# SEEDtk/genome.distance

Hardware: NVIDIA B200
Metric: genome pairs/sec all-vs-all k-mer distance (higher is better)
Workload: dtype u64

## Files before the change

### genome/distance_b200/_lib.py

```python
from __future__ import annotations

import ctypes as C
import os

_HERE = os.path.dirname(os.path.abspath(__file__))
LIB_PATH = os.environ.get("GKD_LIB") or os.path.join(_HERE, "libgkd.so")

GKD_OK, GKD_EINVAL, GKD_EIO, GKD_ENOMEM, GKD_ECUDA, GKD_ESTATE = 0, -1, -2, -3, -4, -5
DNA, PROT, RNA = 0, 1, 2
STRAND_BOTH, STRAND_CANONICAL = 0, 1
AMBIG_SKIP, AMBIG_LITERAL = 0, 1
HASH_JAVA_STRING, HASH_MURMUR3 = 0, 1
ABI_VERSION = 2


class GkdConfig(C.Structure):
    _fields_ = [("device", C.c_int32), ("k", C.c_int32), ("alphabet", C.c_int32), ("strand_mode", C.c_int32),
                ("workspace_bytes", C.c_uint64), ("segment_keys", C.c_uint32), ("ambig_policy", C.c_int32),
                ("reserved", C.c_uint32 * 6)]


class GkdPackedSet(C.Structure):
    _fields_ = [("offs_off", C.c_uint64), ("lows_off", C.c_uint64), ("pal_offs_off", C.c_uint64),
                ("pal_lows_off", C.c_uint64), ("n", C.c_uint32), ("n_pal", C.c_uint32), ("level", C.c_uint32),
# ... 64 lines not shown
    "gkd_query_vs_ref": (_i32, [_vp, _vp, _u32, _vp, _u32, _vp, _vp]),
    "gkd_pairs": (_i32, [_vp, _vp, _vp, _u64, _vp, _vp]),
    "gkd_all_vs_all_range_ex": (_i32, [_vp, _u32, _u64, _u64, C.POINTER(GkdOutputs)]),
    "gkd_query_vs_ref_ex": (_i32, [_vp, _vp, _u32, _vp, _u32, C.POINTER(GkdOutputs)]),
    "gkd_pairs_ex": (_i32, [_vp, _vp, _vp, _u64, C.POINTER(GkdOutputs)]),
    "gkd_greedy_reps": (_i32, [_vp, _vp, _u32, _dbl, _vp]),
    "gkd_pair": (_i32, [_vp, _u32, _u32, _pu64, _pu64, _pdbl]),
    "gkd_all_vs_all_range_within": (_i32, [_vp, _u32, _u64, _u64, _dbl, C.POINTER(GkdHits)]),
    "gkd_query_vs_ref_within": (_i32, [_vp, _vp, _u32, _vp, _u32, _dbl, C.POINTER(GkdHits)]),
    "gkd_query_vs_ref_nearest": (_i32, [_vp, _vp, _u32, _vp, _u32, _u32, _dbl, _i32, _vp, _vp, _vp, _vp]),
    "gkd_hash_set": (_i32, [_vp, _u32, _u32, _i32, _vp, _pu32]),
    "gkd_sketch_distances": (_i32, [_vp, _u32, _i32, _vp, _vp, _u64, _vp]),
    "gkd_format_double": (_i32, [_dbl, C.c_char_p, C.c_size_t]),
    "gkd_get_metrics": (_i32, [_vp, C.POINTER(GkdMetrics)]),
    "gkd_stream": (_vp, [_vp]),
    "gkd_synth_dna": (_i32, [_i32, _vp, _u64, _u64, _u32, _u32, _dbl]),
    "gkd_synth_protein": (_i32, [_i32, _vp, _u64, _u64, _u32, _u32, _dbl]),
}

_lib = None


def load() -> C.CDLL:
    global _lib
    if _lib is not None:
        return _lib
    if not os.path.exists(LIB_PATH):
        raise ImportError(f"{LIB_PATH} is missing: build it with `python -c 'import __graft_entry__ as g; g.build()'` "
                          "(genome.distance_b200 has no CPU fallback)")
    lib = C.CDLL(LIB_PATH)
# ... 7 lines not shown
```

### genome/distance_b200/csrc/gkd_api.cu

```cuda
#include <cuda_runtime.h>
#include <nvtx3/nvToolsExt.h>

#include <algorithm>
#include <cmath>
#include <cstdarg>
#include <cstdio>
#include <cstdlib>
#include <cstring>
#include <new>
#include <string>
#include <unordered_map>
#include <vector>

#include "gkd_internal.cuh"

using namespace gkd;

struct FastaPiece {
    const char *ptr;
    uint64_t len;
};
struct FastaRecord {
    std::string label, comment;
    std::vector<FastaPiece> lines;
// ... 503 lines not shown
    GenomeRec &g = c->genomes[id];
    g.packed = p;
    g.arena = arena_idx;
    set_desc_from_packed(g, base);
    g.built = true;
    c->m.keys_unique += p.n;
}

int build_batch_msd(gkd_ctx *c, const std::vector<BatchGenome> &bg, const std::vector<uint32_t> &ids, uint32_t n_tiles,
                    const uint64_t *keys_in, bool *done) {
    *done = false;
    const uint32_t n = (uint32_t)bg.size();
    std::vector<MsdGenome> msd(n);
    uint32_t n_bins = 0, max_p = 0;
    uint64_t bin_keys = 0;
    bool narrow = true;
    for (uint32_t i = 0; i < n; i++) {
        uint32_t p = level_for(bg[i].n_slots, MSD_BIN_AVG);
        if (bg[i].n_slots >= (1u << 18) && c->key_bits > 32) p = std::max<uint32_t>(p, (uint32_t)c->key_bits - 32);
        p = std::min<uint32_t>(std::min<uint32_t>(p, MSD_MAX_P), (uint32_t)c->key_bits);
        const double mean = (double)bg[i].n_slots / (double)(1u << p);
        uint32_t cap = (uint32_t)(mean + 8.0 * std::sqrt(mean) + 64.0);
        cap = std::min<uint32_t>((cap + 3) & ~3u, MSD_BIN_CAP);
        if (mean > MSD_BIN_AVG) return GKD_OK;
        MsdGenome &M = msd[i];
        M = MsdGenome{};
        M.bin_first = n_bins;
        M.p = p;
        M.s = std::min<uint32_t>(MSD_SORT_BITS, (uint32_t)c->key_bits - p);
        M.cap = cap;
        M.bins_off = bin_keys;
        n_bins += 1u << p;
        bin_keys += (uint64_t)cap << p;
        max_p = std::max(max_p, p);
        narrow = narrow && (c->key_bits - (int)p <= 32);
    }
    int rc;
    if ((rc = ensure(c, c->keys_b, std::max<uint64_t>(bin_keys, 16) * 8))) return rc;
    if ((rc = ensure(c, c->msd_genomes, n * sizeof(MsdGenome)))) return rc;
    if ((rc = ensure(c, c->msd_bins32, (uint64_t)n_bins * 4 + 16))) return rc;
    if ((rc = ensure(c, c->msd_bins64, (uint64_t)n_bins * 8))) return rc;
    if ((rc = ensure(c, c->msd_gstat, (uint64_t)n * 12))) return rc;
    MsdPlan mp{};
    mp.n_bins = n_bins;
    mp.max_p = max_p;
    mp.key_bits = c->key_bits;
    mp.bins = (uint64_t *)c->keys_b.p;
    mp.bin_cursor = (uint32_t *)c->msd_bins32.p;
    mp.overflow = mp.bin_cursor + n_bins;
    mp.status = (unsigned long long *)c->msd_bins64.p;
    mp.genome_valid = (uint32_t *)c->msd_gstat.p;
    mp.genome_maxbin = mp.genome_valid + n;
    mp.genome_unique = mp.genome_maxbin + n;
    CK(cudaMemcpyAsync(c->msd_genomes.p, msd.data(), n * sizeof(MsdGenome), cudaMemcpyHostToDevice, c->stream));
    CK(cudaMemsetAsync(mp.bin_cursor, 0, (size_t)n_bins * 4 + 16, c->stream));
    CK(cudaMemsetAsync(mp.status, 0, (size_t)n_bins * 8, c->stream));
    nvtxRangePushA(keys_in ? "gkd kernel 3: partition into bins" : "gkd kernels 2+3: encode + mix + partition into bins");
    CK(launch_encode_scatter((const BatchGenome *)c->batch_genomes.p, n, n_tiles, (const MsdGenome *)c->msd_genomes.p, max_p,
                             c->cfg.alphabet, c->k, c->mix, keys_in, mp.bins, mp.bin_cursor, mp.overflow, c->stream));
    nvtxRangePop();
    CK(launch_msd_totals((const MsdGenome *)c->msd_genomes.p, n, mp, c->stream));
    c->m.launches += 2;
    std::vector<uint32_t> stat(2 * (size_t)n);
    uint32_t overflow = 0;
    CK(cudaMemcpyAsync(stat.data(), mp.genome_valid, 2 * (size_t)n * 4, cudaMemcpyDeviceToHost, c->stream));
    CK(cudaMemcpyAsync(&overflow, mp.overflow, 4, cudaMemcpyDeviceToHost, c->stream));
    CK(cudaEventRecord(c->ev[1], c->stream));
    CK(cudaEventRecord(c->ev[2], c->stream));
    CK(cudaStreamSynchronize(c->stream));
    if (overflow) return GKD_OK;
    const uint64_t lsz = c->low_bits / 8;
    std::vector<gkd_packed_set> packed(n);
    uint64_t cur = 0;
    for (uint32_t i = 0; i < n; i++) {
// ... 40 lines not shown
int sort_and_finish_lsd(gkd_ctx *c, const std::vector<BatchGenome> &bg, const std::vector<uint32_t> &ids, const SortPlan &plan) {
    uint64_t *sorted = nullptr;
    uint32_t passes = 0;
    nvtxRangePushA("gkd kernel 3: LSD radix sort");
    CK(launch_sort((const BatchGenome *)c->batch_genomes.p, plan, &sorted, &passes, c->stream));
    nvtxRangePop();
    c->m.launches += 3ull * passes;
    c->m.sort_passes = passes;
    CK(cudaEventRecord(c->ev[2], c->stream));
    NvtxRange nvtx("gkd kernel 3: unique + bucket tables");
    return finish_batch(c, bg, ids, plan, sorted);
}

bool msd_applies(const gkd_ctx *c) { return c->use_msd && !has_pal_lists(c); }

int plan_batch(gkd_ctx *c, std::vector<BatchGenome> &bg, SortPlan &plan, uint64_t raw_keys, uint32_t n_tiles) {
    int rc;
    if ((rc = ensure(c, c->keys_a, raw_keys * 8))) return rc;
    if ((rc = ensure(c, c->keys_b, raw_keys * 8))) return rc;
    if ((rc = ensure(c, c->tile_hist, (uint64_t)std::max(n_tiles, 1u) * RADIX_BINS * 4))) return rc;
    if ((rc = ensure(c, c->tile_uniq, (uint64_t)std::max(n_tiles, 1u) * 8))) return rc;
    if ((rc = ensure(c, c->genome_counts, bg.size() * 8))) return rc;
    if ((rc = ensure(c, c->batch_genomes, bg.size() * sizeof(BatchGenome)))) return rc;
    CK(cudaMemcpyAsync(c->batch_genomes.p, bg.data(), bg.size() * sizeof(BatchGenome), cudaMemcpyHostToDevice, c->stream));
    plan.n_genomes = (uint32_t)bg.size();
    plan.n_tiles = n_tiles;
    plan.key_bits = c->key_bits;
    plan.keys_a = (uint64_t *)c->keys_a.p;
    plan.keys_b = (uint64_t *)c->keys_b.p;
    plan.tile_hist = (uint32_t *)c->tile_hist.p;
    plan.tile_uniq = (uint64_t *)c->tile_uniq.p;
    plan.genome_counts = (uint64_t *)c->genome_counts.p;
    return GKD_OK;
}

int build_batch(gkd_ctx *c, uint32_t first, uint32_t last) {
    std::vector<BatchGenome> bg;
    std::vector<uint32_t> ids;
    uint64_t raw = 0;
    uint32_t tiles = 0;
    for (uint32_t id = first; id < last; id++) {
        GenomeRec &g = c->genomes[id];
        BatchGenome b;
        b.codes = (const uint64_t *)g.d_codes;
// ... 3 lines not shown
        b.raw_off = raw;
        b.tile_first = tiles;
        b.n_tiles = (b.n_slots + SORT_TILE - 1) / SORT_TILE;
        raw += ((uint64_t)b.n_slots + 15) & ~15ull;
        tiles += b.n_tiles;
        bg.push_back(b);
        ids.push_back(id);
        c->m.kmer_positions += b.n_slots;
    }
    for (uint32_t id = last; id-- > first;)
        if (c->genomes[id].ready) {
            CK(cudaStreamWaitEvent(c->stream, c->genomes[id].ready, 0));
            break;
        }
    SortPlan plan{};
    int rc = plan_batch(c, bg, plan, std::max<uint64_t>(raw, 16), tiles);
    if (rc) return rc;
    CK(cudaEventRecord(c->ev[0], c->stream));
    c->m.keys_sorted += raw;
    bool done = false;
    if (msd_applies(c)) {
        rc = build_batch_msd(c, bg, ids, tiles, nullptr, &done);
        if (rc) return rc;
        plan.keys_b = (uint64_t *)c->keys_b.p;
    }
    if (!done) {
        nvtxRangePushA("gkd kernel 2: canonical encode + mix");
        CK(launch_encode((const BatchGenome *)c->batch_genomes.p, plan.n_genomes, tiles, c->cfg.alphabet, c->k, c->mix,
                         plan.keys_a, c->stream));
        nvtxRangePop();
        if (tiles) c->m.launches++;
        CK(cudaEventRecord(c->ev[1], c->stream));
        rc = sort_and_finish_lsd(c, bg, ids, plan);
        if (rc) return rc;
    }
    CK(cudaEventRecord(c->ev[3], c->stream));
    CK(cudaStreamSynchronize(c->stream));
    c->m.encode_ms += elapsed(c->ev[0], c->ev[1]);
    c->m.sort_ms += elapsed(c->ev[1], c->ev[2]);
    c->m.unique_ms += elapsed(c->ev[2], c->ev[3]);
    return GKD_OK;
// ... 19 lines not shown
    uint32_t tiles = 0;
    const uint64_t k0 = offsets[i0], total = offsets[i1] - k0;
    for (uint32_t i = i0; i < i1; i++) {
        BatchGenome &b = bg[i - i0];
        b.codes = nullptr;
        b.mask = nullptr;
        b.raw_off = offsets[i] - k0;
        b.n_pos = 0;
        b.n_slots = (uint32_t)(offsets[i + 1] - offsets[i]);
        b.tile_first = tiles;
        b.n_tiles = (b.n_slots + SORT_TILE - 1) / SORT_TILE;
        tiles += b.n_tiles;
        ids[i - i0] = id0 + (i - i0);
    }
    SortPlan plan{};
    int rc = plan_batch(c, bg, plan, std::max<uint64_t>(total, 16), tiles);
    if (rc) return rc;
    if (total) {
        CK(cudaMemcpyAsync(plan.keys_a, keys + k0, total * 8, cudaMemcpyDefault, c->stream));
        if (!on_device) c->m.h2d_bytes += total * 8;
        CK(launch_mix_keys(plan.keys_a, total, c->mix, c->stream));
        c->m.launches++;
    }
    for (uint32_t i = i0; i < i1; i++) c->genomes.push_back(GenomeRec());
    bool done = false;
    rc = GKD_OK;
    if (msd_applies(c)) {
        rc = build_batch_msd(c, bg, ids, tiles, plan.keys_a, &done);
        plan.keys_b = (uint64_t *)c->keys_b.p;
    }
    if (!rc && !done) rc = sort_and_finish_lsd(c, bg, ids, plan);
// ... 805 lines not shown

int gkd_export_set(gkd_ctx *c, uint32_t id, uint64_t *keys, uint64_t cap, uint64_t *n) {
    CHECK_CTX(c);
    int rc = check_built(c, id);
    if (rc) return rc;
    const SetDesc &d = c->genomes[id].desc;
    if (n) *n = d.main.n;
    if (!keys) return GKD_OK;
    if (cap < d.main.n) return fail(c, GKD_EINVAL, "export buffer holds %llu keys, set has %u", (unsigned long long)cap, d.main.n);
    if (d.main.n == 0) return GKD_OK;
    CK(cudaSetDevice(c->cfg.device));
    ABI_GUARD_BEGIN
    std::vector<BatchGenome> bg(1);
    bg[0] = BatchGenome{nullptr, nullptr, 0, 0, d.main.n, 0, (d.main.n + SORT_TILE - 1) / SORT_TILE};
    SortPlan plan{};
    if ((rc = plan_batch(c, bg, plan, d.main.n, bg[0].n_tiles))) return rc;
    CK(launch_unmix_set(d.main, c->mix, c->low_bits, plan.keys_a, c->stream));
    uint64_t *sorted = nullptr;
    uint32_t passes = 0;
    CK(launch_sort((const BatchGenome *)c->batch_genomes.p, plan, &sorted, &passes, c->stream));
    c->m.launches += 1 + 3ull * passes;
    CK(cudaMemcpyAsync(keys, sorted, (uint64_t)d.main.n * 8, cudaMemcpyDefault, c->stream));
    CK(cudaStreamSynchronize(c->stream));
    c->m.d2h_bytes += (uint64_t)d.main.n * 8;
    return GKD_OK;
    ABI_GUARD_END(c)
}

int gkd_import_sets(gkd_ctx *c, const uint64_t *keys, const uint64_t *offsets, uint32_t n_sets, uint32_t *first_id) {
    CHECK_CTX(c);
    if (first_id) *first_id = (uint32_t)c->genomes.size();
// ... 613 lines not shown
    CK(cudaMemcpyAsync(dist, c->d_dist.p, n_pairs * 8, cudaMemcpyDefault, c->stream));
    CK(cudaStreamSynchronize(c->stream));
    c->m.d2h_bytes += n_pairs * 8;
    return GKD_OK;
    ABI_GUARD_END(c)
}

int gkd_get_metrics(const gkd_ctx *c, gkd_metrics *out) {
    if (!c || !out) return GKD_EINVAL;
    *out = c->m;
    return GKD_OK;
}

void *gkd_stream(const gkd_ctx *c) { return c ? (void *)c->stream : nullptr; }

int gkd_format_double(double v, char *buf, size_t cap) {
    if (std::isnan(v)) return snprintf(buf, cap, "NaN");
    if (std::isinf(v)) return snprintf(buf, cap, v > 0 ? "Infinity" : "-Infinity");
    if (v == 0.0) return snprintf(buf, cap, std::signbit(v) ? "-0.0" : "0.0");
    char tmp[48];
    int prec = 17;
    for (int p = 1; p <= 17; p++) {
        snprintf(tmp, sizeof(tmp), "%.*e", p - 1, v);
        if (strtod(tmp, nullptr) == v) {
            prec = p;
            break;
        }
    }
    snprintf(tmp, sizeof(tmp), "%.*e", prec - 1, v);
    std::string mant;
// ... 45 lines not shown
```

### genome/distance_b200/csrc/gkd_internal.cuh

```cuda
#pragma once

#include <cuda_runtime.h>
#include <stdint.h>

#include "gkd.h"

namespace gkd {

constexpr uint64_t KEY_SENTINEL = 0xFFFFFFFFFFFFFFFFull;

struct MixParams {
    uint64_t mask;
    uint64_t fix;
    int bits;
    int shift;
};

constexpr uint64_t MIX_C1 = 0xff51afd7ed558ccdull, MIX_C2 = 0xc4ceb9fe1a85ec53ull;
constexpr uint64_t MIX_I1 = 0x4f74430c22a54005ull, MIX_I2 = 0x9cb4b2f8129337dbull;

__host__ __device__ inline uint64_t mix_rounds(uint64_t x, uint64_t mask, int s) {
    x ^= x >> s;
    x = (x * MIX_C1) & mask;
    x ^= x >> s;
// ... 130 lines not shown
constexpr uint32_t MSD_MAX_P = 12, MSD_SORT_BITS = 12;
struct MsdGenome {
    uint32_t bin_first;
    uint32_t p;
    uint32_t s;
    uint32_t level;
    uint32_t cap;
    uint32_t pad_;
    uint64_t bins_off;
    void *lows;
    uint32_t *offs;
};
struct MsdPlan {
    uint32_t n_bins, max_p;
    int key_bits;
    uint64_t *bins;
    uint32_t *bin_cursor;
    unsigned long long *status;
    uint32_t *genome_valid, *genome_maxbin, *genome_unique, *overflow;
};
cudaError_t msd_configure();
cudaError_t launch_encode_scatter(const BatchGenome *genomes, uint32_t n_genomes, uint32_t n_tiles, const MsdGenome *msd,
                                  uint32_t max_p, int alphabet, int k, MixParams mix, const uint64_t *keys_in, uint64_t *bins_out,
                                  uint32_t *bin_cursor, uint32_t *overflow, cudaStream_t s);
cudaError_t launch_msd_totals(const MsdGenome *msd, uint32_t n_genomes, const MsdPlan &plan, cudaStream_t s);
cudaError_t launch_msd_binsort(const MsdGenome *msd, uint32_t n_genomes, const MsdPlan &plan, int low_bits, bool narrow,
                               cudaStream_t s);
cudaError_t launch_mix_keys(uint64_t *keys, uint64_t n, MixParams mix, cudaStream_t s);
cudaError_t launch_unmix_set(SubSet set, MixParams mix, int low_bits, uint64_t *keys_out, cudaStream_t s);
cudaError_t launch_fill_u64(uint64_t *dst, uint64_t n, uint64_t value, cudaStream_t s);
struct IsectPlan {
    int low_bits;
    uint32_t tmax;
    uint32_t level_min;
    uint32_t groups_per_item;
    uint32_t items_per_pair;
};
cudaError_t intersect_configure();
uint32_t intersect_default_tmax(int low_bits);
// ... 107 lines not shown
```

### genome/distance_b200/csrc/pack_encode.cu

```cuda
#include "gkd_internal.cuh"

namespace gkd {

__device__ __forceinline__ uint32_t nonzero_bytes(uint32_t v) {
    return (((v & 0x7F7F7F7Fu) + 0x7F7F7F7Fu) | v) & 0x80808080u;
}

__global__ void __launch_bounds__(256) k_pack_dna(const char *__restrict__ text, uint64_t n_pos, uint64_t n_words,
                                                   uint64_t *__restrict__ codes, uint32_t *__restrict__ mask, int rna) {
    uint64_t w = (uint64_t)blockIdx.x * blockDim.x + threadIdx.x;
    if (w >= n_words) return;
    uint64_t p0 = w * PACK_POS_PER_WORD;
    uint32_t x[8];
    const char *src = text + p0;
    if (p0 + 32 <= n_pos && ((reinterpret_cast<uintptr_t>(src) & 15) == 0)) {
        uint4 a = __ldg(reinterpret_cast<const uint4 *>(src));
        uint4 b = __ldg(reinterpret_cast<const uint4 *>(src) + 1);
        x[0] = a.x; x[1] = a.y; x[2] = a.z; x[3] = a.w;
        x[4] = b.x; x[5] = b.y; x[6] = b.z; x[7] = b.w;
    } else {
#pragma unroll
        for (int q = 0; q < 8; q++) {
            uint32_t v = 0;
#pragma unroll
// ... 153 lines not shown
        }
#pragma unroll
        for (int u = 0; u < 4; u++) base[u] = v[u] ? atomicAdd(&cursor[b0 + u * ENC_THREADS], v[u]) : 0u;
#pragma unroll
        for (int u = 0; u < 4; u++)
            if (v[u]) {
                if (base[u] + v[u] > cap) {
                    atomicExch(overflow, 1u);
                    base[u] = 0xFFFFFFFFu;
                }
                s_bin[b0 + u * ENC_THREADS] = base[u];
            }
    }
}

template <int ALPHA>
__global__ void __launch_bounds__(ENC_THREADS, 4)
    k_encode_scatter(const BatchGenome *__restrict__ genomes, uint32_t n_genomes, const MsdGenome *__restrict__ msd, int k,
                     MixParams mix, uint64_t *__restrict__ bins_out, uint32_t *__restrict__ bin_cursor,
                     uint32_t *__restrict__ overflow) {
    extern __shared__ uint32_t s_bin[];
    __shared__ uint32_t s_g;
    if (threadIdx.x == 0) s_g = find_genome(genomes, n_genomes, blockIdx.x);
    __syncthreads();
    const BatchGenome G = genomes[s_g];
    const MsdGenome M = msd[s_g];
    const uint32_t n_bins = 1u << M.p;
    for (uint32_t i = threadIdx.x; i < n_bins; i += ENC_THREADS) s_bin[i] = 0;
    __syncthreads();
    const int shift = mix.bits - (int)M.p;
    const uint32_t my0 = (blockIdx.x - G.tile_first) * ENC_TILE + threadIdx.x * ENC_PER_THREAD;
    uint64_t key[ENC_PER_THREAD];
    uint32_t rank[ENC_PER_THREAD];
#pragma unroll
    for (int j = 0; j < ENC_PER_THREAD; j++) key[j] = KEY_SENTINEL, rank[j] = 0;
    if (my0 < G.n_slots)
        encode_thread<ALPHA>(G, k, mix, my0, [&](int j, uint64_t h) {
            key[j] = h;
            if (h != KEY_SENTINEL) rank[j] = atomicAdd(&s_bin[M.p ? (uint32_t)(h >> shift) : 0u], 1u);
        });
    __syncthreads();
    reserve_bins(s_bin, n_bins, bin_cursor + M.bin_first, M.cap, overflow);
    __syncthreads();
    uint64_t *out = bins_out + M.bins_off;
#pragma unroll
    for (int j = 0; j < ENC_PER_THREAD; j++)
        if (key[j] != KEY_SENTINEL) {
            const uint32_t b = M.p ? (uint32_t)(key[j] >> shift) : 0u;
            const uint32_t base = s_bin[b];
            if (base != 0xFFFFFFFFu) out[(uint64_t)b * M.cap + base + rank[j]] = key[j];
        }
}

__global__ void __launch_bounds__(ENC_THREADS)
    k_keys_scatter(const BatchGenome *__restrict__ genomes, uint32_t n_genomes, const MsdGenome *__restrict__ msd, int key_bits,
                   const uint64_t *__restrict__ in, uint64_t *__restrict__ bins_out, uint32_t *__restrict__ bin_cursor,
                   uint32_t *__restrict__ overflow) {
    extern __shared__ uint32_t s_bin[];
    __shared__ uint32_t s_g;
    if (threadIdx.x == 0) s_g = find_genome(genomes, n_genomes, blockIdx.x);
    __syncthreads();
    const BatchGenome G = genomes[s_g];
    const MsdGenome M = msd[s_g];
    const uint32_t n_bins = 1u << M.p;
    for (uint32_t i = threadIdx.x; i < n_bins; i += ENC_THREADS) s_bin[i] = 0;
    __syncthreads();
    const int shift = key_bits - (int)M.p;
    const uint32_t slot0 = (blockIdx.x - G.tile_first) * ENC_TILE;
    const uint32_t count = min((uint32_t)ENC_TILE, G.n_slots - slot0);
    const uint64_t *src = in + G.raw_off + slot0;
    uint64_t key[ENC_PER_THREAD];
    uint32_t rank[ENC_PER_THREAD];
#pragma unroll
    for (int j = 0; j < ENC_PER_THREAD; j++) {
        const uint32_t idx = j * ENC_THREADS + threadIdx.x;
        key[j] = idx < count ? src[idx] : KEY_SENTINEL;
        rank[j] = 0;
        if (key[j] != KEY_SENTINEL) rank[j] = atomicAdd(&s_bin[M.p ? (uint32_t)(key[j] >> shift) : 0u], 1u);
    }
    __syncthreads();
    reserve_bins(s_bin, n_bins, bin_cursor + M.bin_first, M.cap, overflow);
    __syncthreads();
    uint64_t *out = bins_out + M.bins_off;
#pragma unroll
    for (int j = 0; j < ENC_PER_THREAD; j++)
        if (key[j] != KEY_SENTINEL) {
            const uint32_t b = M.p ? (uint32_t)(key[j] >> shift) : 0u;
            const uint32_t base = s_bin[b];
            if (base != 0xFFFFFFFFu) out[(uint64_t)b * M.cap + base + rank[j]] = key[j];
        }
}

cudaError_t launch_encode(const BatchGenome *genomes, uint32_t n_genomes, uint32_t n_tiles, int alphabet, int k,
                          MixParams mix, uint64_t *keys_out, cudaStream_t s) {
    if (n_tiles == 0) return cudaSuccess;
    if (alphabet == GKD_PROT) k_encode<GKD_PROT><<<n_tiles, ENC_THREADS, 0, s>>>(genomes, n_genomes, k, mix, keys_out);
    else k_encode<GKD_DNA><<<n_tiles, ENC_THREADS, 0, s>>>(genomes, n_genomes, k, mix, keys_out);
    return cudaGetLastError();
}

}

namespace gkd {

cudaError_t launch_encode_scatter(const BatchGenome *genomes, uint32_t n_genomes, uint32_t n_tiles, const MsdGenome *msd,
                                  uint32_t max_p, int alphabet, int k, MixParams mix, const uint64_t *keys_in, uint64_t *bins_out,
                                  uint32_t *bin_cursor, uint32_t *overflow, cudaStream_t s) {
    if (n_tiles == 0) return cudaSuccess;
    const uint32_t smem = (1u << max_p) * 4;
    if (keys_in)
        k_keys_scatter<<<n_tiles, ENC_THREADS, smem, s>>>(genomes, n_genomes, msd, mix.bits, keys_in, bins_out, bin_cursor, overflow);
    else if (alphabet == GKD_PROT)
        k_encode_scatter<GKD_PROT><<<n_tiles, ENC_THREADS, smem, s>>>(genomes, n_genomes, msd, k, mix, bins_out, bin_cursor, overflow);
    else
        k_encode_scatter<GKD_DNA><<<n_tiles, ENC_THREADS, smem, s>>>(genomes, n_genomes, msd, k, mix, bins_out, bin_cursor, overflow);
    return cudaGetLastError();
}

}
```

### genome/distance_b200/csrc/sort_msd.cu

```cuda
#include "gkd_internal.cuh"

namespace gkd {

constexpr int MSD_THREADS = 512;
constexpr int MSD_KPT = (MSD_BIN_CAP + MSD_THREADS - 1) / MSD_THREADS;

__global__ void __launch_bounds__(256)
    k_msd_totals(const MsdGenome *__restrict__ msd, const uint32_t *__restrict__ bin_cursor,
                 uint32_t *__restrict__ genome_valid, uint32_t *__restrict__ genome_maxbin) {
    __shared__ uint32_t s_sum, s_max;
    const MsdGenome M = msd[blockIdx.x];
    if (threadIdx.x == 0) s_sum = 0, s_max = 0;
    __syncthreads();
    uint32_t sum = 0, mx = 0;
    for (uint32_t b = threadIdx.x; b < (1u << M.p); b += 256) {
        const uint32_t v = bin_cursor[M.bin_first + b];
        sum += v;
        mx = v > mx ? v : mx;
    }
    sum = __reduce_add_sync(0xffffffffu, sum);
    mx = __reduce_max_sync(0xffffffffu, mx);
    if ((threadIdx.x & 31) == 0) {
        atomicAdd(&s_sum, sum);
        atomicMax(&s_max, mx);
// ... 20 lines not shown
    for (int w = 0; w < MSD_THREADS / 32; w++) {
        const uint32_t c = s_warp[w];
        if (w < warp) base += c;
        tot += c;
    }
    *total = tot;
    __syncthreads();
    return base + incl - v;
}

constexpr unsigned long long LB_AGG = 1ull << 62, LB_PREFIX = 2ull << 62, LB_MASK = (1ull << 62) - 1;

template <typename KT, typename LowT>
__global__ void __launch_bounds__(MSD_THREADS, 2)
    k_msd_binsort(const MsdGenome *__restrict__ msd, uint32_t n_genomes, int key_bits, const uint32_t *__restrict__ bin_cursor,
                  const uint64_t *__restrict__ bins, unsigned long long *__restrict__ status,
                  uint32_t *__restrict__ genome_unique) {
    extern __shared__ __align__(16) unsigned char s_raw[];
    KT *s_k = reinterpret_cast<KT *>(s_raw);
    KT *s_o = s_k + MSD_BIN_CAP;
    uint32_t *s_cnt = reinterpret_cast<uint32_t *>(s_o + MSD_BIN_CAP);
    uint32_t *s_start = s_cnt + (1u << MSD_SORT_BITS);
    __shared__ uint32_t s_warp[MSD_THREADS / 32];
    __shared__ unsigned long long s_prefix;
    uint32_t lo = 0, hi = n_genomes;
    while (hi - lo > 1) {
        const uint32_t mid = (lo + hi) >> 1;
        if (msd[mid].bin_first <= blockIdx.x) lo = mid;
        else hi = mid;
    }
    const MsdGenome M = msd[lo];
    const uint32_t bin = blockIdx.x - M.bin_first, n_bins = 1u << M.p;
    uint32_t c = bin_cursor[blockIdx.x];
    if (c > M.cap || c > MSD_BIN_CAP) c = 0;
    const uint64_t *src = bins + M.bins_off + (uint64_t)bin * M.cap;
    const int rest = key_bits - (int)M.p;
    const uint64_t rest_mask = rest >= 64 ? ~0ull : ((1ull << rest) - 1ull);
    const uint32_t s = M.s, n_sb = 1u << s;
    const int sb_shift = rest - (int)s;

    for (uint32_t i = threadIdx.x; i < n_sb; i += MSD_THREADS) s_cnt[i] = 0;
    __syncthreads();
    KT kv[MSD_KPT];
    uint32_t meta[MSD_KPT];
    const int rounds = (int)((c + MSD_THREADS - 1) / MSD_THREADS);
    uint64_t raw[MSD_KPT];
#pragma unroll
    for (int j = 0; j < MSD_KPT; j++) {
        if (j >= rounds) break;
        const uint32_t i = j * MSD_THREADS + threadIdx.x;
        raw[j] = i < c ? src[i] : 0ull;
    }
#pragma unroll
    for (int j = 0; j < MSD_KPT; j++) {
        if (j >= rounds) break;
        const uint32_t i = j * MSD_THREADS + threadIdx.x;
        kv[j] = 0;
        meta[j] = 0;
        if (i < c) {
            const uint64_t h = raw[j] & rest_mask;
            const uint32_t sb = s ? (uint32_t)(h >> sb_shift) : 0u;
            kv[j] = (KT)h;
            meta[j] = sb | (atomicAdd(&s_cnt[sb], 1u) << 16);
        }
    }
    __syncthreads();
    {
        constexpr uint32_t SB_PT = (1u << MSD_SORT_BITS) / MSD_THREADS;
        static_assert(SB_PT * MSD_THREADS == (1u << MSD_SORT_BITS) && SB_PT >= 1, "whole sort-buckets per thread");
        const uint32_t a = SB_PT * threadIdx.x;
        uint32_t v[SB_PT], sum = 0, total;
#pragma unroll
        for (uint32_t q = 0; q < SB_PT; q++) {
            v[q] = a + q < n_sb ? s_cnt[a + q] : 0u;
            sum += v[q];
// ... 84 lines not shown
    }
    if (bin == n_bins - 1 && threadIdx.x == 0) {
        M.offs[(size_t)1 << M.level] = prefix + u;
        genome_unique[lo] = prefix + u;
    }
}

template <typename KT>
static constexpr uint32_t binsort_smem() { return 2 * MSD_BIN_CAP * (uint32_t)sizeof(KT) + (2 * (1u << MSD_SORT_BITS) + 8) * 4; }

cudaError_t msd_configure() {
    cudaError_t e;
#define X(KT, LT)                                                                                                  \
    if ((e = cudaFuncSetAttribute(k_msd_binsort<KT, LT>, cudaFuncAttributeMaxDynamicSharedMemorySize, (int)binsort_smem<KT>()))) \
        return e;
    X(uint32_t, uint32_t) X(uint64_t, uint32_t) X(uint64_t, uint64_t)
#undef X
    return cudaSuccess;
}

cudaError_t launch_msd_totals(const MsdGenome *msd, uint32_t n_genomes, const MsdPlan &plan, cudaStream_t s) {
    if (n_genomes == 0) return cudaSuccess;
    k_msd_totals<<<n_genomes, 256, 0, s>>>(msd, plan.bin_cursor, plan.genome_valid, plan.genome_maxbin);
    return cudaGetLastError();
}

cudaError_t launch_msd_binsort(const MsdGenome *msd, uint32_t n_genomes, const MsdPlan &plan, int low_bits, bool narrow,
                               cudaStream_t s) {
    if (plan.n_bins == 0) return cudaSuccess;
    if (low_bits == 32 && narrow)
        k_msd_binsort<uint32_t, uint32_t><<<plan.n_bins, MSD_THREADS, binsort_smem<uint32_t>(), s>>>(
            msd, n_genomes, plan.key_bits, plan.bin_cursor, plan.bins, plan.status, plan.genome_unique);
    else if (low_bits == 32)
        k_msd_binsort<uint64_t, uint32_t><<<plan.n_bins, MSD_THREADS, binsort_smem<uint64_t>(), s>>>(
            msd, n_genomes, plan.key_bits, plan.bin_cursor, plan.bins, plan.status, plan.genome_unique);
    else
        k_msd_binsort<uint64_t, uint64_t><<<plan.n_bins, MSD_THREADS, binsort_smem<uint64_t>(), s>>>(
            msd, n_genomes, plan.key_bits, plan.bin_cursor, plan.bins, plan.status, plan.genome_unique);
    return cudaGetLastError();
}

}
```

### genome/distance_b200/engine.py

```python
from __future__ import annotations

import ctypes as C
from typing import List, Sequence, Tuple

import numpy as np

from . import _lib
from ._lib import (AMBIG_LITERAL, AMBIG_SKIP, DNA, PROT, RNA, STRAND_BOTH, STRAND_CANONICAL, GkdConfig, GkdHits,
                   GkdMetrics, GkdOutputs, GkdPackedSet)

PACKED_DTYPE = np.dtype([("offs_off", "<u8"), ("lows_off", "<u8"), ("pal_offs_off", "<u8"), ("pal_lows_off", "<u8"),
                         ("n", "<u4"), ("n_pal", "<u4"), ("level", "<u4"), ("pal_level", "<u4")])
assert PACKED_DTYPE.itemsize == C.sizeof(GkdPackedSet)


FIRST_HITS_CAP = 1 << 20


def _select(call, pairs: int):
    cap = min(pairs, FIRST_HITS_CAP)
    while True:
        a, b = np.empty(cap, dtype=np.uint32), np.empty(cap, dtype=np.uint32)
        inter, dist = np.empty(cap, dtype=np.uint64), np.empty(cap, dtype=np.float64)
        h = GkdHits(a.ctypes.data, b.ctypes.data, inter.ctypes.data, dist.ctypes.data, cap, 0)
# ... 18 lines not shown
class Engine:

    def __init__(self, k: int = 0, alphabet: int = DNA, strand_mode: int = STRAND_BOTH, device: int = 0,
                 workspace_bytes: int = 0, segment_keys: int = 0, ambig_policy: int = AMBIG_SKIP):
        self._L = _lib.load()
        cfg = GkdConfig(device=device, k=k, alphabet=alphabet, strand_mode=strand_mode,
                        workspace_bytes=workspace_bytes, segment_keys=segment_keys, ambig_policy=ambig_policy)
        h = C.c_void_p()
        rc = self._L.gkd_create(C.byref(h), C.byref(cfg))
        if rc:
            raise GkdError(rc, (self._L.gkd_last_error(None) or b"").decode())
        self._h = h
        self.device = device
        self.alphabet = alphabet
        self._keep: List[object] = []
        self._adopted: List[Tuple[int, object]] = []

    def _ck(self, rc: int):
        if rc:
            raise GkdError(rc, (self._L.gkd_last_error(self._h) or b"").decode())

    def close(self):
        if getattr(self, "_h", None):
            self._L.gkd_destroy(self._h)
            self._h = None

    def __del__(self):
        try:
            self.close()
        except Exception:
# ... 19 lines not shown
            t = x.contiguous()
            return t.data_ptr(), t.numel() * t.element_size(), t
        raise TypeError(f"unsupported sequence type {type(x)}")

    def add(self, contigs) -> int:
        if isinstance(contigs, (str, bytes, bytearray, np.ndarray)) or _is_torch(contigs):
            contigs = [contigs]
        triples = [self._ptr_len(c) for c in contigs]
        n = len(triples)
        ptrs = (C.c_void_p * max(n, 1))(*[t[0] for t in triples])
        lens = (C.c_uint64 * max(n, 1))(*[t[1] for t in triples])
        out = C.c_uint32()
        if any(_is_torch(c) and c.is_cuda for c in contigs):
            import torch

            torch.cuda.synchronize(self.device)
        self._ck(self._L.gkd_add_sequences(self._h, ptrs, lens, n, C.byref(out)))
        self._keep.extend(t[2] for t in triples if _is_torch(t[2]))
        return out.value

    def add_fasta(self, path: str, per_record: bool = True) -> Tuple[int, int]:
        first, n = C.c_uint32(), C.c_uint32()
        self._ck(self._L.gkd_add_fasta_file(self._h, path.encode(), 1 if per_record else 0, C.byref(first), C.byref(n)))
        return first.value, n.value

    def label(self, i: int) -> str:
        return self._L.gkd_label(self._h, i).decode("latin-1")

    def comment(self, i: int) -> str:
        return self._L.gkd_comment(self._h, i).decode("latin-1")

# ... 299 lines not shown
```

### include/gkd.h

```cpp
#ifndef GKD_H
#define GKD_H

#include <stddef.h>
#include <stdint.h>

#ifdef __cplusplus
extern "C" {
#endif

#define GKD_ABI_VERSION 2

typedef enum gkd_status {
    GKD_OK = 0,
    GKD_EINVAL = -1,
    GKD_EIO = -2,
    GKD_ENOMEM = -3,
    GKD_ECUDA = -4,
    GKD_ESTATE = -5
} gkd_status;

typedef enum gkd_alphabet { GKD_DNA = 0, GKD_PROT = 1, GKD_RNA = 2 } gkd_alphabet;

typedef enum gkd_strand_mode { GKD_STRAND_BOTH = 0, GKD_STRAND_CANONICAL = 1 } gkd_strand_mode;

// ... 117 lines not shown
int gkd_group_add_fasta_file(gkd_group *g, const char *path, uint32_t *n_added);
const char *gkd_group_label(const gkd_group *g, uint32_t global_id);
const char *gkd_group_comment(const gkd_group *g, uint32_t global_id);
int gkd_group_build(gkd_group *g);
int gkd_group_all_vs_all(gkd_group *g, uint64_t *inter, double *dist);
int gkd_group_all_vs_all_within(gkd_group *g, double max_dist, gkd_hits *out);

typedef enum gkd_sketch_hash { GKD_HASH_JAVA_STRING = 0, GKD_HASH_MURMUR3 = 1 } gkd_sketch_hash;
int gkd_hash_set(gkd_ctx *ctx, uint32_t id, uint32_t width, int hash, int32_t *out, uint32_t *n_out);
int gkd_sketch_distances(gkd_ctx *ctx, uint32_t width, int hash, const uint32_t *a, const uint32_t *b, uint64_t n_pairs,
                         double *dist);

int gkd_format_double(double v, char *buf, size_t cap);
int gkd_get_metrics(const gkd_ctx *ctx, gkd_metrics *out);
void *gkd_stream(const gkd_ctx *ctx);

int gkd_synth_dna(int device, char *dst, uint64_t len, uint64_t seed, uint32_t family, uint32_t member,
                  double sub_rate);
int gkd_synth_protein(int device, char *dst, uint64_t len, uint64_t seed, uint32_t family, uint32_t member,
                      double sub_rate);

#ifdef __cplusplus
}
#endif
#endif
```

Before: 1.394 million.

## Store narrow MSD bin keys as 32-bit and replace host sync with event wait

When every genome's post-bin remainder fits in 32 bits, the encode/scatter kernels now write only the masked low bits into 32-bit bin buffers, and the binsort kernel reads them as uint32 (a new uint32/uint64 instantiation is added). This halves scatter and binsort global memory traffic and the size of the keys_b allocation, and LSD key buffers are now allocated only when the MSD path does not finish the batch. Separately, adding CUDA-tensor contigs no longer calls a full device synchronize; it records a torch event and makes the library streams wait on it. The risks are correctness in the masking and narrow logic, plus ordering subtleties from the asynchronous handoff.

```diff
diff --git a/genome/distance_b200/_lib.py b/genome/distance_b200/_lib.py
--- a/genome/distance_b200/_lib.py
+++ b/genome/distance_b200/_lib.py
@@ -102,6 +102,7 @@
     "gkd_format_double": (_i32, [_dbl, C.c_char_p, C.c_size_t]),
     "gkd_get_metrics": (_i32, [_vp, C.POINTER(GkdMetrics)]),
     "gkd_stream": (_vp, [_vp]),
+    "gkd_wait_event": (_i32, [_vp, _vp]),
     "gkd_synth_dna": (_i32, [_i32, _vp, _u64, _u64, _u32, _u32, _dbl]),
     "gkd_synth_protein": (_i32, [_i32, _vp, _u64, _u64, _u32, _u32, _dbl]),
 }
diff --git a/genome/distance_b200/csrc/gkd_api.cu b/genome/distance_b200/csrc/gkd_api.cu
--- a/genome/distance_b200/csrc/gkd_api.cu
+++ b/genome/distance_b200/csrc/gkd_api.cu
@@ -541,11 +541,15 @@
     std::vector<MsdGenome> msd(n);
     uint32_t n_bins = 0, max_p = 0;
     uint64_t bin_keys = 0;
-    bool narrow = true;
-    for (uint32_t i = 0; i < n; i++) {
+    auto bin_bits = [&](uint32_t i) {
         uint32_t p = level_for(bg[i].n_slots, MSD_BIN_AVG);
         if (bg[i].n_slots >= (1u << 18) && c->key_bits > 32) p = std::max<uint32_t>(p, (uint32_t)c->key_bits - 32);
-        p = std::min<uint32_t>(std::min<uint32_t>(p, MSD_MAX_P), (uint32_t)c->key_bits);
+        return std::min<uint32_t>(std::min<uint32_t>(p, MSD_MAX_P), (uint32_t)c->key_bits);
+    };
+    bool narrow = true;
+    for (uint32_t i = 0; i < n; i++) narrow = narrow && (c->key_bits - (int)bin_bits(i) <= 32);
+    for (uint32_t i = 0; i < n; i++) {
+        const uint32_t p = bin_bits(i);
         const double mean = (double)bg[i].n_slots / (double)(1u << p);
         uint32_t cap = (uint32_t)(mean + 8.0 * std::sqrt(mean) + 64.0);
         cap = std::min<uint32_t>((cap + 3) & ~3u, MSD_BIN_CAP);
@@ -560,10 +564,9 @@
         n_bins += 1u << p;
         bin_keys += (uint64_t)cap << p;
         max_p = std::max(max_p, p);
-        narrow = narrow && (c->key_bits - (int)p <= 32);
     }
     int rc;
-    if ((rc = ensure(c, c->keys_b, std::max<uint64_t>(bin_keys, 16) * 8))) return rc;
+    if ((rc = ensure(c, c->keys_b, std::max<uint64_t>(bin_keys, 16) * (narrow ? 4 : 8)))) return rc;
     if ((rc = ensure(c, c->msd_genomes, n * sizeof(MsdGenome)))) return rc;
     if ((rc = ensure(c, c->msd_bins32, (uint64_t)n_bins * 4 + 16))) return rc;
     if ((rc = ensure(c, c->msd_bins64, (uint64_t)n_bins * 8))) return rc;
@@ -572,7 +575,7 @@
     mp.n_bins = n_bins;
     mp.max_p = max_p;
     mp.key_bits = c->key_bits;
-    mp.bins = (uint64_t *)c->keys_b.p;
+    mp.bins = c->keys_b.p;
     mp.bin_cursor = (uint32_t *)c->msd_bins32.p;
     mp.overflow = mp.bin_cursor + n_bins;
     mp.status = (unsigned long long *)c->msd_bins64.p;
@@ -584,7 +587,8 @@
     CK(cudaMemsetAsync(mp.status, 0, (size_t)n_bins * 8, c->stream));
     nvtxRangePushA(keys_in ? "gkd kernel 3: partition into bins" : "gkd kernels 2+3: encode + mix + partition into bins");
     CK(launch_encode_scatter((const BatchGenome *)c->batch_genomes.p, n, n_tiles, (const MsdGenome *)c->msd_genomes.p, max_p,
-                             c->cfg.alphabet, c->k, c->mix, keys_in, mp.bins, mp.bin_cursor, mp.overflow, c->stream));
+                             narrow, c->cfg.alphabet, c->k, c->mix, keys_in, c->keys_b.p, mp.bin_cursor, mp.overflow,
+                             c->stream));
     nvtxRangePop();
     CK(launch_msd_totals((const MsdGenome *)c->msd_genomes.p, n, mp, c->stream));
     c->m.launches += 2;
@@ -655,10 +659,17 @@
 
 bool msd_applies(const gkd_ctx *c) { return c->use_msd && !has_pal_lists(c); }
 
-int plan_batch(gkd_ctx *c, std::vector<BatchGenome> &bg, SortPlan &plan, uint64_t raw_keys, uint32_t n_tiles) {
+int plan_lsd_keys(gkd_ctx *c, SortPlan &plan, uint64_t raw_keys) {
     int rc;
     if ((rc = ensure(c, c->keys_a, raw_keys * 8))) return rc;
     if ((rc = ensure(c, c->keys_b, raw_keys * 8))) return rc;
+    plan.keys_a = (uint64_t *)c->keys_a.p;
+    plan.keys_b = (uint64_t *)c->keys_b.p;
+    return GKD_OK;
+}
+
+int plan_batch(gkd_ctx *c, std::vector<BatchGenome> &bg, SortPlan &plan, uint32_t n_tiles) {
+    int rc;
     if ((rc = ensure(c, c->tile_hist, (uint64_t)std::max(n_tiles, 1u) * RADIX_BINS * 4))) return rc;
     if ((rc = ensure(c, c->tile_uniq, (uint64_t)std::max(n_tiles, 1u) * 8))) return rc;
     if ((rc = ensure(c, c->genome_counts, bg.size() * 8))) return rc;
@@ -667,8 +678,6 @@
     plan.n_genomes = (uint32_t)bg.size();
     plan.n_tiles = n_tiles;
     plan.key_bits = c->key_bits;
-    plan.keys_a = (uint64_t *)c->keys_a.p;
-    plan.keys_b = (uint64_t *)c->keys_b.p;
     plan.tile_hist = (uint32_t *)c->tile_hist.p;
     plan.tile_uniq = (uint64_t *)c->tile_uniq.p;
     plan.genome_counts = (uint64_t *)c->genome_counts.p;
@@ -702,7 +711,7 @@
             break;
         }
     SortPlan plan{};
-    int rc = plan_batch(c, bg, plan, std::max<uint64_t>(raw, 16), tiles);
+    int rc = plan_batch(c, bg, plan, tiles);
     if (rc) return rc;
     CK(cudaEventRecord(c->ev[0], c->stream));
     c->m.keys_sorted += raw;
@@ -710,9 +719,9 @@
     if (msd_applies(c)) {
         rc = build_batch_msd(c, bg, ids, tiles, nullptr, &done);
         if (rc) return rc;
-        plan.keys_b = (uint64_t *)c->keys_b.p;
     }
     if (!done) {
+        if ((rc = plan_lsd_keys(c, plan, std::max<uint64_t>(raw, 16)))) return rc;
         nvtxRangePushA("gkd kernel 2: canonical encode + mix");
         CK(launch_encode((const BatchGenome *)c->batch_genomes.p, plan.n_genomes, tiles, c->cfg.alphabet, c->k, c->mix,
                          plan.keys_a, c->stream));
@@ -762,7 +771,8 @@
         ids[i - i0] = id0 + (i - i0);
     }
     SortPlan plan{};
-    int rc = plan_batch(c, bg, plan, std::max<uint64_t>(total, 16), tiles);
+    int rc = plan_batch(c, bg, plan, tiles);
+    if (!rc) rc = plan_lsd_keys(c, plan, std::max<uint64_t>(total, 16));
     if (rc) return rc;
     if (total) {
         CK(cudaMemcpyAsync(plan.keys_a, keys + k0, total * 8, cudaMemcpyDefault, c->stream));
@@ -1598,7 +1608,7 @@
     std::vector<BatchGenome> bg(1);
     bg[0] = BatchGenome{nullptr, nullptr, 0, 0, d.main.n, 0, (d.main.n + SORT_TILE - 1) / SORT_TILE};
     SortPlan plan{};
-    if ((rc = plan_batch(c, bg, plan, d.main.n, bg[0].n_tiles))) return rc;
+    if ((rc = plan_batch(c, bg, plan, bg[0].n_tiles)) || (rc = plan_lsd_keys(c, plan, d.main.n))) return rc;
     CK(launch_unmix_set(d.main, c->mix, c->low_bits, plan.keys_a, c->stream));
     uint64_t *sorted = nullptr;
     uint32_t passes = 0;
@@ -2242,6 +2252,14 @@
 
 void *gkd_stream(const gkd_ctx *c) { return c ? (void *)c->stream : nullptr; }
 
+int gkd_wait_event(gkd_ctx *c, void *event) {
+    if (!c || !event) return GKD_EINVAL;
+    CK(cudaSetDevice(c->cfg.device));
+    CK(cudaStreamWaitEvent(c->copy_stream, (cudaEvent_t)event, 0));
+    CK(cudaStreamWaitEvent(c->stream, (cudaEvent_t)event, 0));
+    return GKD_OK;
+}
+
 int gkd_format_double(double v, char *buf, size_t cap) {
     if (std::isnan(v)) return snprintf(buf, cap, "NaN");
     if (std::isinf(v)) return snprintf(buf, cap, v > 0 ? "Infinity" : "-Infinity");
diff --git a/genome/distance_b200/csrc/gkd_internal.cuh b/genome/distance_b200/csrc/gkd_internal.cuh
--- a/genome/distance_b200/csrc/gkd_internal.cuh
+++ b/genome/distance_b200/csrc/gkd_internal.cuh
@@ -168,15 +168,15 @@
 struct MsdPlan {
     uint32_t n_bins, max_p;
     int key_bits;
-    uint64_t *bins;
+    const void *bins;
     uint32_t *bin_cursor;
     unsigned long long *status;
     uint32_t *genome_valid, *genome_maxbin, *genome_unique, *overflow;
 };
 cudaError_t msd_configure();
 cudaError_t launch_encode_scatter(const BatchGenome *genomes, uint32_t n_genomes, uint32_t n_tiles, const MsdGenome *msd,
-                                  uint32_t max_p, int alphabet, int k, MixParams mix, const uint64_t *keys_in, uint64_t *bins_out,
-                                  uint32_t *bin_cursor, uint32_t *overflow, cudaStream_t s);
+                                  uint32_t max_p, bool narrow, int alphabet, int k, MixParams mix, const uint64_t *keys_in,
+                                  void *bins_out, uint32_t *bin_cursor, uint32_t *overflow, cudaStream_t s);
 cudaError_t launch_msd_totals(const MsdGenome *msd, uint32_t n_genomes, const MsdPlan &plan, cudaStream_t s);
 cudaError_t launch_msd_binsort(const MsdGenome *msd, uint32_t n_genomes, const MsdPlan &plan, int low_bits, bool narrow,
                                cudaStream_t s);
diff --git a/genome/distance_b200/csrc/pack_encode.cu b/genome/distance_b200/csrc/pack_encode.cu
--- a/genome/distance_b200/csrc/pack_encode.cu
+++ b/genome/distance_b200/csrc/pack_encode.cu
@@ -191,10 +191,10 @@
     }
 }
 
-template <int ALPHA>
+template <int ALPHA, typename KT>
 __global__ void __launch_bounds__(ENC_THREADS, 4)
     k_encode_scatter(const BatchGenome *__restrict__ genomes, uint32_t n_genomes, const MsdGenome *__restrict__ msd, int k,
-                     MixParams mix, uint64_t *__restrict__ bins_out, uint32_t *__restrict__ bin_cursor,
+                     MixParams mix, KT *__restrict__ bins_out, uint32_t *__restrict__ bin_cursor,
                      uint32_t *__restrict__ overflow) {
     extern __shared__ uint32_t s_bin[];
     __shared__ uint32_t s_g;
@@ -219,19 +219,21 @@
     __syncthreads();
     reserve_bins(s_bin, n_bins, bin_cursor + M.bin_first, M.cap, overflow);
     __syncthreads();
-    uint64_t *out = bins_out + M.bins_off;
+    const uint64_t rest_mask = shift >= 64 ? ~0ull : ((1ull << shift) - 1ull);
+    KT *out = bins_out + M.bins_off;
 #pragma unroll
     for (int j = 0; j < ENC_PER_THREAD; j++)
         if (key[j] != KEY_SENTINEL) {
             const uint32_t b = M.p ? (uint32_t)(key[j] >> shift) : 0u;
             const uint32_t base = s_bin[b];
-            if (base != 0xFFFFFFFFu) out[(uint64_t)b * M.cap + base + rank[j]] = key[j];
-        }
-}
-
+            if (base != 0xFFFFFFFFu) out[(uint64_t)b * M.cap + base + rank[j]] = (KT)(key[j] & rest_mask);
+        }
+}
+
+template <typename KT>
 __global__ void __launch_bounds__(ENC_THREADS)
     k_keys_scatter(const BatchGenome *__restrict__ genomes, uint32_t n_genomes, const MsdGenome *__restrict__ msd, int key_bits,
-                   const uint64_t *__restrict__ in, uint64_t *__restrict__ bins_out, uint32_t *__restrict__ bin_cursor,
+                   const uint64_t *__restrict__ in, KT *__restrict__ bins_out, uint32_t *__restrict__ bin_cursor,
                    uint32_t *__restrict__ overflow) {
     extern __shared__ uint32_t s_bin[];
     __shared__ uint32_t s_g;
@@ -258,13 +260,14 @@
     __syncthreads();
     reserve_bins(s_bin, n_bins, bin_cursor + M.bin_first, M.cap, overflow);
     __syncthreads();
-    uint64_t *out = bins_out + M.bins_off;
+    const uint64_t rest_mask = shift >= 64 ? ~0ull : ((1ull << shift) - 1ull);
+    KT *out = bins_out + M.bins_off;
 #pragma unroll
     for (int j = 0; j < ENC_PER_THREAD; j++)
         if (key[j] != KEY_SENTINEL) {
             const uint32_t b = M.p ? (uint32_t)(key[j] >> shift) : 0u;
             const uint32_t base = s_bin[b];
-            if (base != 0xFFFFFFFFu) out[(uint64_t)b * M.cap + base + rank[j]] = key[j];
+            if (base != 0xFFFFFFFFu) out[(uint64_t)b * M.cap + base + rank[j]] = (KT)(key[j] & rest_mask);
         }
 }
 
@@ -280,18 +283,29 @@
 
 namespace gkd {
 
-cudaError_t launch_encode_scatter(const BatchGenome *genomes, uint32_t n_genomes, uint32_t n_tiles, const MsdGenome *msd,
-                                  uint32_t max_p, int alphabet, int k, MixParams mix, const uint64_t *keys_in, uint64_t *bins_out,
-                                  uint32_t *bin_cursor, uint32_t *overflow, cudaStream_t s) {
-    if (n_tiles == 0) return cudaSuccess;
+template <typename KT>
+static cudaError_t encode_scatter_t(const BatchGenome *genomes, uint32_t n_genomes, uint32_t n_tiles, const MsdGenome *msd,
+                                    uint32_t max_p, int alphabet, int k, MixParams mix, const uint64_t *keys_in, KT *bins_out,
+                                    uint32_t *bin_cursor, uint32_t *overflow, cudaStream_t s) {
     const uint32_t smem = (1u << max_p) * 4;
     if (keys_in)
-        k_keys_scatter<<<n_tiles, ENC_THREADS, smem, s>>>(genomes, n_genomes, msd, mix.bits, keys_in, bins_out, bin_cursor, overflow);
+        k_keys_scatter<KT><<<n_tiles, ENC_THREADS, smem, s>>>(genomes, n_genomes, msd, mix.bits, keys_in, bins_out, bin_cursor, overflow);
     else if (alphabet == GKD_PROT)
-        k_encode_scatter<GKD_PROT><<<n_tiles, ENC_THREADS, smem, s>>>(genomes, n_genomes, msd, k, mix, bins_out, bin_cursor, overflow);
+        k_encode_scatter<GKD_PROT, KT><<<n_tiles, ENC_THREADS, smem, s>>>(genomes, n_genomes, msd, k, mix, bins_out, bin_cursor, overflow);
     else
-        k_encode_scatter<GKD_DNA><<<n_tiles, ENC_THREADS, smem, s>>>(genomes, n_genomes, msd, k, mix, bins_out, bin_cursor, overflow);
+        k_encode_scatter<GKD_DNA, KT><<<n_tiles, ENC_THREADS, smem, s>>>(genomes, n_genomes, msd, k, mix, bins_out, bin_cursor, overflow);
     return cudaGetLastError();
 }
 
-}
+cudaError_t launch_encode_scatter(const BatchGenome *genomes, uint32_t n_genomes, uint32_t n_tiles, const MsdGenome *msd,
+                                  uint32_t max_p, bool narrow, int alphabet, int k, MixParams mix, const uint64_t *keys_in,
+                                  void *bins_out, uint32_t *bin_cursor, uint32_t *overflow, cudaStream_t s) {
+    if (n_tiles == 0) return cudaSuccess;
+    if (narrow)
+        return encode_scatter_t<uint32_t>(genomes, n_genomes, n_tiles, msd, max_p, alphabet, k, mix, keys_in,
+                                          (uint32_t *)bins_out, bin_cursor, overflow, s);
+    return encode_scatter_t<uint64_t>(genomes, n_genomes, n_tiles, msd, max_p, alphabet, k, mix, keys_in,
+                                      (uint64_t *)bins_out, bin_cursor, overflow, s);
+}
+
+}
diff --git a/genome/distance_b200/csrc/sort_msd.cu b/genome/distance_b200/csrc/sort_msd.cu
--- a/genome/distance_b200/csrc/sort_msd.cu
+++ b/genome/distance_b200/csrc/sort_msd.cu
@@ -58,7 +58,7 @@
 template <typename KT, typename LowT>
 __global__ void __launch_bounds__(MSD_THREADS, 2)
     k_msd_binsort(const MsdGenome *__restrict__ msd, uint32_t n_genomes, int key_bits, const uint32_t *__restrict__ bin_cursor,
-                  const uint64_t *__restrict__ bins, unsigned long long *__restrict__ status,
+                  const KT *__restrict__ bins, unsigned long long *__restrict__ status,
                   uint32_t *__restrict__ genome_unique) {
     extern __shared__ __align__(16) unsigned char s_raw[];
     KT *s_k = reinterpret_cast<KT *>(s_raw);
@@ -77,7 +77,7 @@
     const uint32_t bin = blockIdx.x - M.bin_first, n_bins = 1u << M.p;
     uint32_t c = bin_cursor[blockIdx.x];
     if (c > M.cap || c > MSD_BIN_CAP) c = 0;
-    const uint64_t *src = bins + M.bins_off + (uint64_t)bin * M.cap;
+    const KT *src = bins + M.bins_off + (uint64_t)bin * M.cap;
     const int rest = key_bits - (int)M.p;
     const uint64_t rest_mask = rest >= 64 ? ~0ull : ((1ull << rest) - 1ull);
     const uint32_t s = M.s, n_sb = 1u << s;
@@ -88,12 +88,12 @@
     KT kv[MSD_KPT];
     uint32_t meta[MSD_KPT];
     const int rounds = (int)((c + MSD_THREADS - 1) / MSD_THREADS);
-    uint64_t raw[MSD_KPT];
+    KT raw[MSD_KPT];
 #pragma unroll
     for (int j = 0; j < MSD_KPT; j++) {
         if (j >= rounds) break;
         const uint32_t i = j * MSD_THREADS + threadIdx.x;
-        raw[j] = i < c ? src[i] : 0ull;
+        raw[j] = i < c ? src[i] : (KT)0;
     }
 #pragma unroll
     for (int j = 0; j < MSD_KPT; j++) {
@@ -102,7 +102,7 @@
         kv[j] = 0;
         meta[j] = 0;
         if (i < c) {
-            const uint64_t h = raw[j] & rest_mask;
+            const uint64_t h = (uint64_t)raw[j] & rest_mask;
             const uint32_t sb = s ? (uint32_t)(h >> sb_shift) : 0u;
             kv[j] = (KT)h;
             meta[j] = sb | (atomicAdd(&s_cnt[sb], 1u) << 16);
@@ -217,7 +217,7 @@
 #define X(KT, LT)                                                                                                  \
     if ((e = cudaFuncSetAttribute(k_msd_binsort<KT, LT>, cudaFuncAttributeMaxDynamicSharedMemorySize, (int)binsort_smem<KT>()))) \
         return e;
-    X(uint32_t, uint32_t) X(uint64_t, uint32_t) X(uint64_t, uint64_t)
+    X(uint32_t, uint32_t) X(uint32_t, uint64_t) X(uint64_t, uint32_t) X(uint64_t, uint64_t)
 #undef X
     return cudaSuccess;
 }
@@ -233,13 +233,16 @@
     if (plan.n_bins == 0) return cudaSuccess;
     if (low_bits == 32 && narrow)
         k_msd_binsort<uint32_t, uint32_t><<<plan.n_bins, MSD_THREADS, binsort_smem<uint32_t>(), s>>>(
-            msd, n_genomes, plan.key_bits, plan.bin_cursor, plan.bins, plan.status, plan.genome_unique);
+            msd, n_genomes, plan.key_bits, plan.bin_cursor, (const uint32_t *)plan.bins, plan.status, plan.genome_unique);
+    else if (narrow)
+        k_msd_binsort<uint32_t, uint64_t><<<plan.n_bins, MSD_THREADS, binsort_smem<uint32_t>(), s>>>(
+            msd, n_genomes, plan.key_bits, plan.bin_cursor, (const uint32_t *)plan.bins, plan.status, plan.genome_unique);
     else if (low_bits == 32)
         k_msd_binsort<uint64_t, uint32_t><<<plan.n_bins, MSD_THREADS, binsort_smem<uint64_t>(), s>>>(
-            msd, n_genomes, plan.key_bits, plan.bin_cursor, plan.bins, plan.status, plan.genome_unique);
+            msd, n_genomes, plan.key_bits, plan.bin_cursor, (const uint64_t *)plan.bins, plan.status, plan.genome_unique);
     else
         k_msd_binsort<uint64_t, uint64_t><<<plan.n_bins, MSD_THREADS, binsort_smem<uint64_t>(), s>>>(
-            msd, n_genomes, plan.key_bits, plan.bin_cursor, plan.bins, plan.status, plan.genome_unique);
+            msd, n_genomes, plan.key_bits, plan.bin_cursor, (const uint64_t *)plan.bins, plan.status, plan.genome_unique);
     return cudaGetLastError();
 }
 
diff --git a/genome/distance_b200/engine.py b/genome/distance_b200/engine.py
--- a/genome/distance_b200/engine.py
+++ b/genome/distance_b200/engine.py
@@ -56,6 +56,7 @@
         self.device = device
         self.alphabet = alphabet
         self._keep: List[object] = []
+        self._text_ev = None
         self._adopted: List[Tuple[int, object]] = []
 
     def _ck(self, rc: int):
@@ -105,7 +106,10 @@
         if any(_is_torch(c) and c.is_cuda for c in contigs):
             import torch
 
-            torch.cuda.synchronize(self.device)
+            if self._text_ev is None:
+                self._text_ev = torch.cuda.Event()
+            self._text_ev.record(torch.cuda.current_stream(self.device))
+            self._ck(self._L.gkd_wait_event(self._h, self._text_ev.cuda_event))
         self._ck(self._L.gkd_add_sequences(self._h, ptrs, lens, n, C.byref(out)))
         self._keep.extend(t[2] for t in triples if _is_torch(t[2]))
         return out.value
diff --git a/include/gkd.h b/include/gkd.h
--- a/include/gkd.h
+++ b/include/gkd.h
@@ -155,6 +155,7 @@
 int gkd_format_double(double v, char *buf, size_t cap);
 int gkd_get_metrics(const gkd_ctx *ctx, gkd_metrics *out);
 void *gkd_stream(const gkd_ctx *ctx);
+int gkd_wait_event(gkd_ctx *ctx, void *event);
 
 int gkd_synth_dna(int device, char *dst, uint64_t len, uint64_t seed, uint32_t family, uint32_t member,
                   double sub_rate);
```

Measured after the change: 1.473 million, median of 6. 1.06x the previous value.
